# shg8/3DGS.cpp

Hardware: AMD Instinct MI355X
Metric: frames/sec at 1920×1080, 1M Gaussians (higher is better)
Workload: dtype f32

## Files before the change

### 3dgs.cpp_amd/binding.py

```python
import ctypes as C
import os

import numpy as np

_HERE = os.path.dirname(os.path.abspath(__file__))
LIB_PATH = os.environ.get("GS3D_HIP_LIB", os.path.join(_HERE, "libgs3d_hip.so"))

UNIFORMS_DT = np.dtype([("camera_position", "<f4", 4), ("proj_mat", "<f4", 16), ("view_mat", "<f4", 16),
                        ("width", "<u4"), ("height", "<u4"), ("tan_fovx", "<f4"), ("tan_fovy", "<f4")])
CAMERA_DT = np.dtype([("position", "<f4", 3), ("rotation", "<f4", 4), ("fov", "<f4"),
                      ("near_plane", "<f4"), ("far_plane", "<f4")])
VERTEX_FLOATS = 60
RECORD_FLOATS = 62
BLOB_PLANES = 59


KERNEL_SOURCES = ("gs_device.h", "gs_bin.h", "gs_scene.hip", "gs_preprocess.hip", "gs_radix.hip", "gs_bin_l1.hip", "gs_bin_l2.hip",
                  "gs_blend.hip", "gs_kernels.h")


def library_source_hash():
    import hashlib
    import re
    h = hashlib.sha256()
# ... 7 lines not shown
            text = re.sub(r"#[^\n]*", " ", text)
        h.update(name.encode() + b"\0" + " ".join(text.split()).encode())
    return h.hexdigest()


STAGES = dict(tiles=(0, np.uint32), depth=(1, np.float32), radius=(2, np.float32), aabb=(3, np.uint16),
              conic_opacity=(4, np.float32), uv_rg=(5, np.float32), b=(6, np.float32),
              depth_order=(7, np.uint32), alpha_cut=(8, np.float32), sorted_tile=(11, np.uint32), sorted_gid=(12, np.uint32),
              ranges=(13, np.uint32), lists_raw=(14, np.uint32), ranges_raw=(15, np.uint32))

SYMBOLS = ["gs_last_error", "gs_device_count", "gs_read_ply", "gs_activate_records", "gs_scene_load_ply", "gs_scene_from_records",
           "gs_scene_from_vertices", "gs_scene_from_device_blob", "gs_scene_blob_floats", "gs_scene_blob",
           "gs_scene_num_vertices", "gs_scene_quantize_sh", "gs_scene_sh_bits", "gs_scene_download_vertex_range",
           "gs_scene_download_vertices", "gs_scene_download_cov3d",
           "gs_scene_destroy", "gs_renderer_create", "gs_renderer_destroy", "gs_camera_uniforms",
           "gs_render", "gs_render_host", "gs_synchronize", "gs_set_timing", "gs_set_frames_in_flight", "gs_set_sort_path", "gs_set_exp_mode", "gs_set_graph_mode", "gs_set_blend_lockstep", "gs_get_blend_lockstep", "gs_set_blend_contraction", "gs_set_antialiased", "gs_get_antialiased", "gs_get_timing_totals",
           "gs_get_frame_intervals", "gs_get_stats", "gs_poll_stats", "gs_debug_download", "gs_debug_expf_scan", "gs_debug_alpha_cut_scan", "gs_renderer_stream",
           "gs_dist_unique_id", "gs_dist_create", "gs_dist_rank", "gs_dist_world", "gs_dist_pose_count",
           "gs_dist_broadcast_scene", "gs_dist_broadcast_scene_ex", "gs_dist_verify", "gs_dist_destroy"]


class FrameStats(C.Structure):
    _fields_ = [("num_gaussians", C.c_uint64), ("num_visible", C.c_uint64), ("num_instances", C.c_uint64),
                ("instance_capacity", C.c_uint64), ("ms_preprocess", C.c_float), ("ms_prefix_sum", C.c_float),
                ("ms_preprocess_sort", C.c_float), ("ms_sort", C.c_float), ("ms_tile_boundary", C.c_float),
                ("ms_render", C.c_float), ("ms_total", C.c_float), ("retries", C.c_uint32),
                ("num_bin_entries", C.c_uint32), ("max_bin_entries", C.c_uint32), ("sort_path", C.c_uint32),
                ("bin_tiles", C.c_uint32), ("sort_level", C.c_uint32), ("blend_redo", C.c_uint32), ("blend_resolved", C.c_uint32), ("pad_", C.c_uint32)]

    def as_dict(self):
        return {k: getattr(self, k) for k, _ in self._fields_}
# ... 27 lines not shown
    if _LIB is None:
        if not os.path.exists(LIB_PATH):
            raise GsError(-3, f"{LIB_PATH} is missing: run __graft_entry__.build() (hipcc, gfx950)")
        L = C.CDLL(LIB_PATH)
        L.gs_last_error.restype = C.c_char_p
        L.gs_scene_num_vertices.restype = C.c_uint64
        L.gs_scene_num_vertices.argtypes = [C.c_void_p]
        L.gs_scene_blob_floats.restype = C.c_uint64
        L.gs_scene_blob_floats.argtypes = [C.c_uint64]
        L.gs_renderer_stream.restype = C.c_void_p
        L.gs_renderer_stream.argtypes = [C.c_void_p]
        L.gs_scene_destroy.argtypes = [C.c_void_p]
        L.gs_renderer_destroy.argtypes = [C.c_void_p]
        L.gs_scene_destroy.restype = None
        L.gs_renderer_destroy.restype = None
        _LIB = L
    return _LIB


def _check(rc):
    if rc != 0:
        raise GsError(rc, lib().gs_last_error().decode(errors="replace"))


def _p(a):
    if not isinstance(a, np.ndarray) or not a.flags["C_CONTIGUOUS"]:
        raise TypeError("_p() takes a C-contiguous numpy array that the caller keeps alive for the duration of the call")
    return C.c_void_p(a.ctypes.data)


# ... 137 lines not shown

    def set_exp_mode(self, mode):
        _check(lib().gs_set_exp_mode(self._h, C.c_int(int(mode))))

    def set_blend_contraction(self, enabled):
        _check(lib().gs_set_blend_contraction(self._h, C.c_int(int(bool(enabled)))))

    def set_antialiased(self, enabled):
        _check(lib().gs_set_antialiased(self._h, C.c_int(int(bool(enabled)))))

    @property
    def antialiased(self):
        rc = lib().gs_get_antialiased(self._h)
        _check(min(rc, 0))
        return bool(rc)

    def set_fast_blend(self, fast):
        self.set_exp_mode(0 if fast else 2)
        self.set_blend_contraction(bool(fast))

    def set_graph_mode(self, enabled):
        _check(lib().gs_set_graph_mode(self._h, C.c_int(int(bool(enabled)))))

    def set_blend_lockstep(self, mode):
        _check(lib().gs_set_blend_lockstep(self._h, C.c_int(int(mode))))

    def blend_lockstep(self):
        settled = C.c_int(0)
        now = lib().gs_get_blend_lockstep(self._h, C.byref(settled))
        if now < 0:
# ... 105 lines not shown
```

### 3dgs.cpp_amd/csrc/gs_blend.hip

```cpp
#include "gs_device.h"

namespace gs {

#ifndef GS_BLEND_ASM_ACCUMULATE
#define GS_BLEND_ASM_ACCUMULATE 1
#endif
#ifndef GS_BLEND_ASM_LOOP
#define GS_BLEND_ASM_LOOP 1
#endif
#ifndef GS_BLEND_SALU_DIET
#define GS_BLEND_SALU_DIET 2
#endif


__device__ __forceinline__ float min_q_rect(float c00, float c01, float c11, float u, float v, float xa,
                                            float xb, float ya, float yb) {
    const float dx_lo = u - xb, dx_hi = u - xa, dy_lo = v - yb, dy_hi = v - ya;
    const bool in_x = !(dx_lo > 0.0f) && !(dx_hi < 0.0f), in_y = !(dy_lo > 0.0f) && !(dy_hi < 0.0f);
    const float h00 = 0.5f * c00, h11 = 0.5f * c11;
    const float r11 = -c01 * __builtin_amdgcn_rcpf(c11), r00 = -c01 * __builtin_amdgcn_rcpf(c00);
    const float a = dx_lo > 0.0f ? dx_lo : dx_hi;
    const float t = fminf(fmaxf(r11 * a, dy_lo), dy_hi);
    const float qv = __builtin_fmaf(t, __builtin_fmaf(h11, t, c01 * a), h00 * a * a);
    const float b = dy_lo > 0.0f ? dy_lo : dy_hi;
// ... 518 lines not shown
                if (alive == 0) bm = 0;
#endif
            }
        }
        }
        if (alive == 0) break;
        if (GUARD) {
            S += __builtin_fmaf(T_cs * 1.00001f, __builtin_amdgcn_rcpf(T), -1.0f);
            T_cs = T;
        }
    }
    STAT_ADD(7, (unsigned long long)__popcll(alive) * (range.y - range.x));
    return !abandon;
}

template <int EXP, bool CONTRACT, bool GUARD>
__global__ __launch_bounds__(BLOCK) __attribute__((amdgpu_waves_per_eu(8, 8))) void k_blend(const uint2* __restrict__ ranges,
                                                 const uint32_t* __restrict__ sorted_gid,
                                                 const uint32_t* __restrict__ tile_order,
                                                 const AttrRecord* __restrict__ rec,
                                                 uint32_t width, uint32_t height, uint32_t tiles_x,
                                                 float4* __restrict__ rgba, uchar4* __restrict__ bgra,
                                                 Counters* __restrict__ counters, Counters* host_counters,
                                                 const FrameParams* __restrict__ fp, uint32_t* __restrict__ vis_count, uint32_t lockstep,
                                                 uint64_t* __restrict__ stamps) {
    frame_stamp(stamps, ST_BLEND);
#if defined(GS_BLEND_STATS) || defined(GS_BLEND_CLOCK)
    const long long stat_c0 = clock64();
    const unsigned long long stat_w0 = wall_clock64();
#endif
    static_assert(!GUARD || (EXP != 2 && !CONTRACT), "the guard belongs to a fast exp on the uncontracted arithmetic");
    if (fp) {
        rgba = reinterpret_cast<float4*>(fp->rgba);
        bgra = reinterpret_cast<uchar4*>(fp->bgra);
        host_counters = fp->host_counters;
    }
    __shared__ float4 s_rec[4][3][WAVE];
    __shared__ uint2 s_exptab[(EXP == 2 || GUARD) ? 4 : 1][32];
    __shared__ uint32_t s_klist[GUARD ? 4 : 1][GUARD ? kGuardList : 1];

    const int tid = threadIdx.x, lane = tid & (WAVE - 1), w = tid / WAVE;
    if (EXP == 2) {
        if (lane < 32) {
            const uint64_t v = kExpfTab[lane];
            s_exptab[w][lane] = make_uint2((uint32_t)v, (uint32_t)(v >> 32));
        }
        __builtin_amdgcn_wave_barrier();
    }
    if (host_counters && blockIdx.x == 0 && tid == 0) *host_counters = *counters;
    if (vis_count && blockIdx.x == 0 && (uint32_t)tid < kVisRegions) {
// ... 39 lines not shown
        if ((threadIdx.x & (WAVE - 1)) == 0 && slot < kClockSlots)
            g_blend_clock[slot] = make_uint2((uint32_t)(clock64() - stat_c0), (uint32_t)(wall_clock64() - stat_w0));
    }
#endif
    if (inside) {
        const size_t p = (size_t)py * width + px;
        if (rgba) rgba[p] = make_float4(c0, c1, c2, 1.0f);
        if (bgra) {
            const float r = fminf(fmaxf(c0, 0.0f), 1.0f), g = fminf(fmaxf(c1, 0.0f), 1.0f),
                        b = fminf(fmaxf(c2, 0.0f), 1.0f);
            bgra[p] = make_uchar4((unsigned char)(int)__builtin_rintf(b * 255.0f),
                                  (unsigned char)(int)__builtin_rintf(g * 255.0f),
                                  (unsigned char)(int)__builtin_rintf(r * 255.0f), 255);
        }
    }
}

template <int EXP, bool CONTRACT, bool GUARD>
static void launch_blend_as(const uint32_t* ranges, const uint32_t* sorted_gid, const uint32_t* tile_order, const AttrView& av,
                            uint32_t width, uint32_t height, uint32_t tx, uint32_t ty, float* rgba, uint8_t* bgra,
                            Counters* counters, Counters* host_counters, const FrameParams* fp, bool lockstep, uint64_t* stamps, hipStream_t s) {
    hipLaunchKernelGGL((k_blend<EXP, CONTRACT, GUARD>), dim3(tx * ty), dim3(BLOCK), 0, s, reinterpret_cast<const uint2*>(ranges),
                       sorted_gid, tile_order, av.rec, width, height, tx, reinterpret_cast<float4*>(rgba),
                       reinterpret_cast<uchar4*>(bgra), counters, host_counters, fp, av.vis_count, lockstep ? 1u : 0u, stamps);
}

__global__ __launch_bounds__(WAVE) void k_frame_end(uint64_t* __restrict__ stamps, uint64_t* host_stamps, const FrameParams* __restrict__ fp) {
    if (fp) host_stamps = fp->host_stamps;
    const uint64_t now = wall_clock64();
    const int t = threadIdx.x;
    if (t < ST_COUNT) {
        const uint64_t v = t == ST_END ? now : stamps[t];
        if (t == ST_END) stamps[t] = now;
        if (host_stamps) host_stamps[t] = v;
    }
}
void launch_frame_end(uint64_t* stamps, uint64_t* host_stamps, const FrameParams* fp, hipStream_t s) {
    if (!stamps) return;
    hipLaunchKernelGGL(k_frame_end, dim3(1), dim3(WAVE), 0, s, stamps, host_stamps, fp);
}

void launch_blend(const uint32_t* ranges, const uint32_t* sorted_gid, const uint32_t* tile_order, const AttrView& av,
                  uint32_t width,
                  uint32_t height, float* rgba, uint8_t* bgra, Counters* counters,
                  Counters* host_counters, int exp_mode, bool contract, const FrameParams* fp, bool lockstep, uint64_t* stamps, hipStream_t s) {
    if (width == 0 || height == 0) return;
    const uint32_t tx = (width + kTile - 1) / kTile, ty = (height + kTile - 1) / kTile;
    if (exp_mode == 3 && !contract)
        return launch_blend_as<1, false, true>(ranges, sorted_gid, tile_order, av, width, height, tx, ty, rgba, bgra, counters,
                                               host_counters, fp, lockstep, stamps, s);
    if (exp_mode == 3) exp_mode = 1;
#define GS_BLEND_CASE(E, C)                                                                                              \
    if (exp_mode == E && contract == C)                                                                                  \
        return launch_blend_as<E, C, false>(ranges, sorted_gid, tile_order, av, width, height, tx, ty, rgba, bgra,       \
                                            counters, host_counters, fp, lockstep, stamps, s)
    GS_BLEND_CASE(0, true);
    GS_BLEND_CASE(0, false);
    GS_BLEND_CASE(1, true);
    GS_BLEND_CASE(1, false);
    GS_BLEND_CASE(2, true);
    GS_BLEND_CASE(2, false);
#undef GS_BLEND_CASE
}


__global__ __launch_bounds__(BLOCK) void k_expf_scan(uint32_t first_bits, uint64_t count, unsigned long long* __restrict__ block_sums,
                                                     unsigned long long* __restrict__ guard_max ) {
    const uint64_t base = (uint64_t)blockIdx.x << 20;
    unsigned long long sum = 0;
    double worst = 0.0, worst_near = 0.0;
// ... 76 lines not shown
```

### 3dgs.cpp_amd/csrc/gs_kernels.h

```cpp
#pragma once
#include <hip/hip_runtime.h>
#include <stdint.h>

#include "../../include/gs3d_hip.h"

namespace gs {

constexpr int kTile = 16;
constexpr int kSortTileKeys = 2048;
constexpr int kSortMaxBlocks = 1024;

enum ScenePlane { P_POS = 0, P_SCALE = 3, P_ROT = 6, P_OPACITY = 10, P_SH = 11, P_COUNT = 59 };
constexpr uint64_t blob_stride(uint64_t n) { return (n + 15) & ~uint64_t(15); }
constexpr uint64_t blob_floats(uint64_t n) { return P_SH * blob_stride(n) + 48 * n; }

struct SceneView {
    const float* blob;
    const float* cov3d;
    uint32_t n;
    uint32_t stride;
    const uint16_t* sh16;
    const float* acut;
    const uint32_t* perm;
};
// ... 16 lines not shown
    uint32_t vis_region_slots;
};
constexpr uint32_t kVisRegions = 256, kVisCounterStride = 32;
uint32_t vis_region_slots(uint32_t n);

struct Counters {
    uint32_t visible;
    uint32_t instances;
    uint32_t overflow;
    uint32_t bin_entries;
    uint32_t max_bin;
    uint32_t slabs;
    uint32_t blend_resolved;
    uint32_t blend_redo;
    uint32_t q_head, q_bins_done;
};
enum FrameStamp { ST_PREPROCESS = 0, ST_ORDER = 1, ST_L1_COUNT = 2, ST_L1_SCATTER = 3, ST_L2 = 4, ST_BLEND = 5, ST_END = 6, ST_COUNT = 8 };

struct FrameParams {
    gs_uniforms u;
    float* rgba;
    uint8_t* bgra;
    Counters* host_counters;
    uint64_t* host_stamps;
};

constexpr int kBinSortLevels = 5;
constexpr int kBinSlabLevel = 4;
constexpr uint32_t kBinSortLimit[kBinSortLevels] = {4096, 8192, 12288, 16384, 65535};
constexpr int kBinSortMax = 16384;
constexpr uint32_t kSlabDescBytes = 288, kSlabCapacity = 8192, kSlabWorkGroups = 512, kQueueWorkGroups = 256;

void launch_cov3d(const float* blob, float* cov3d, uint32_t n, uint32_t stride, hipStream_t s);
void launch_alpha_cut(const float* blob, float* cut, uint32_t n, uint32_t stride, uint32_t* beyond_unit, hipStream_t s);
void launch_permute_blob(const float* src, const uint32_t* perm, float* dst, uint32_t n, uint32_t stride, hipStream_t s);
void launch_blob_checksum(const float* blob, uint64_t floats, uint64_t* out, hipStream_t s);
void launch_sh_to_half(const float* blob, uint16_t* sh16, uint32_t n, uint32_t stride, hipStream_t s);
void launch_preprocess(const SceneView& sv, const gs_uniforms& u, const AttrView& av, Counters* counters,
                       const FrameParams* fp, uint64_t* stamps, bool antialiased, hipStream_t s);
// ... 50 lines not shown
void bin_debug_occupancy();
hipError_t bin_prepare_device();
void launch_bin_level1_count(const BinLaunch& b, hipStream_t s);
void launch_bin_level1_scatter(const BinLaunch& b, bool any_order, hipStream_t s);
void launch_bin_level2(const BinLaunch& b, int level, hipStream_t s);

void launch_blend(const uint32_t* ranges, const uint32_t* sorted_gid, const uint32_t* tile_order, const AttrView& av,
                  uint32_t width,
                  uint32_t height, float* rgba, uint8_t* bgra, Counters* counters,
                  Counters* host_counters ,
                  int exp_mode ,
                  bool contract ,
                  const FrameParams* fp,
                  bool lockstep ,
                  uint64_t* stamps ,
                  hipStream_t s);

}
```

### 3dgs.cpp_amd/csrc/gs_preprocess.hip

```cpp
#include "gs_device.h"

namespace gs {

#ifndef GS_PRE_AA_BISECT
#define GS_PRE_AA_BISECT 0
#endif

#ifndef GS_PRE_SH_LDS
#define GS_PRE_SH_LDS 1
#endif

constexpr float SH_C0 = 0.28209479177387814f;
constexpr float SH_C1 = 0.4886025119029199f;

__device__ __forceinline__ float ndc2pix(float v, int S) { return ((v + 1.0f) * (float)S - 1.0f) * 0.5f; }

struct PreUniforms {
    gs_uniforms u;
    Counters* counters;
    const FrameParams* fp;
    uint64_t* stamps;
};

constexpr int kPrePlane = 68, kPreStage = 3 * kPrePlane + 16;
// ... 324 lines not shown
    __shared__ float4 s_stage[BLOCK / WAVE][kPreWaveLds];
    const gs_uniforms& u = pu.fp ? pu.fp->u : pu.u;
    const uint32_t i = blockIdx.x * BLOCK + threadIdx.x;
    frame_stamp(pu.stamps, ST_PREPROCESS);
    if (i == 0 && pu.counters) {
        pu.counters->visible = 0;
        pu.counters->instances = 0;
        pu.counters->overflow = 0;
        pu.counters->bin_entries = 0;
        pu.counters->max_bin = 0;
        pu.counters->slabs = 0;
        pu.counters->blend_resolved = 0;
        pu.counters->blend_redo = 0;
        pu.counters->q_head = 0;
        pu.counters->q_bins_done = 0;
    }
    preprocess_one<AA>(sv, u, av, i, i < sv.n, s_stage[threadIdx.x / WAVE]);
}

void launch_preprocess(const SceneView& sv, const gs_uniforms& u, const AttrView& av, Counters* counters,
                       const FrameParams* fp, uint64_t* stamps, bool antialiased, hipStream_t s) {
    if (sv.n == 0) return;
    PreUniforms pu;
    pu.u = u;
    pu.counters = counters;
    pu.fp = fp;
    pu.stamps = stamps;
    if (antialiased)
        hipLaunchKernelGGL(k_preprocess<true>, dim3((sv.n + BLOCK - 1) / BLOCK), dim3(BLOCK), 0, s, sv, pu, av);
    else
// ... 4 lines not shown
```

### 3dgs.cpp_amd/csrc/gs_renderer.cpp

```cpp
#include <algorithm>
#include <chrono>
#include <cstdio>
#include <cstdlib>
#include <cstring>
#include <limits>
#include <memory>
#include <string>
#include <vector>

#include "gs_blend_tuner.h"
#include "gs_internal.h"

using namespace gs_host;

#ifndef GS_L1_DENSE
#define GS_L1_DENSE 1
#endif
struct FrameBuffers {
    hipStream_t stream = nullptr;
    hipStream_t blend_stream = nullptr;
    hipEvent_t prep_done = nullptr, blend_done = nullptr;
    bool blend_recorded = false;
    DevBuf<uint32_t> tiles;
    DevBuf<float> depth;
    DevBuf<ushort4> aabb;
    DevBuf<gs::AttrRecord> rec;
    DevBuf<uint4> vis;
    DevBuf<uint32_t> vis_count;
    bool planes_stale = false;
    uint32_t vis_region_slots = 0;
    DevBuf<uint32_t> dkeys[2], dvals[2];
    DevBuf<uint32_t> block_hist, digit_total;
    DevBuf<uint32_t> l1_hist, bin_count;
    DevBuf<uint32_t> cand;
    DevBuf<uint32_t> sorted;
// ... 14 lines not shown
                   capacity == o.capacity && cand_capacity == o.cand_capacity && tile_order == o.tile_order && ranges == o.ranges && sh16 == o.sh16;
        }
    } graph_keys[2];
    void drop_graph(int which) {
        if (graph_execs[which]) (void)hipGraphExecDestroy(graph_execs[which]);
        graph_execs[which] = nullptr;
        graph_keys[which] = GraphKey{};
    }
    void drop_graph() {
        drop_graph(0);
        drop_graph(1);
    }
    size_t n = 0;
    bool ready = false;

    void init(size_t n_, uint32_t capacity, uint32_t cand_capacity, const std::vector<uint32_t>& mask_prep, const std::vector<uint32_t>& mask_blend, bool dense_lists) {
        n = n_;
        if (!mask_prep.empty() && !mask_blend.empty()) {
            HIP_CHECK(hipExtStreamCreateWithCUMask(&stream, static_cast<uint32_t>(mask_prep.size()), mask_prep.data()));
            HIP_CHECK(hipExtStreamCreateWithCUMask(&blend_stream, static_cast<uint32_t>(mask_blend.size()), mask_blend.data()));
            HIP_CHECK(hipEventCreateWithFlags(&prep_done, hipEventDisableTiming));
            HIP_CHECK(hipEventCreateWithFlags(&blend_done, hipEventDisableTiming));
        } else {
            HIP_CHECK(hipStreamCreateWithFlags(&stream, hipStreamNonBlocking));
        }
        tiles.alloc(n);
        depth.alloc(n);
        aabb.alloc(n);
        rec.alloc(n);
        vis_region_slots = gs::vis_region_slots(static_cast<uint32_t>(n));
        if (dense_lists) ensure_dense_lists();
        l1_hist.alloc(1025 * static_cast<size_t>(gs::bin_level1_columns(static_cast<uint32_t>(n))));
        bin_count.alloc(2048);
        counters.alloc(1);
        stamps.alloc(gs::ST_COUNT);
        HIP_CHECK(hipMemset(stamps.p, 0, gs::ST_COUNT * sizeof(uint64_t)));
        params.alloc(1);
        set_capacity(capacity);
        set_cand_capacity(cand_capacity);
        ready = true;
// ... 15 lines not shown
    }
    void set_capacity(uint32_t cap) {
        drop_graph();
        sorted.alloc(static_cast<size_t>(cap) + 4);
    }
    void set_cand_capacity(uint32_t ccap) {
        drop_graph();
        cand.alloc(3 * static_cast<size_t>(ccap));
        HIP_CHECK(hipMemset(cand.p, 0, 3 * static_cast<size_t>(ccap) * sizeof(uint32_t)));
    }
    void sync() const {
        HIP_CHECK(hipStreamSynchronize(stream));
        if (blend_stream) HIP_CHECK(hipStreamSynchronize(blend_stream));
    }
    ~FrameBuffers() {
        drop_graph();
        if (stream) (void)hipStreamDestroy(stream);
        if (blend_stream) (void)hipStreamDestroy(blend_stream);
        if (prep_done) (void)hipEventDestroy(prep_done);
        if (blend_done) (void)hipEventDestroy(blend_done);
    }
};

struct FrameSlot {
    gs_uniforms u{};
    float* rgba = nullptr;
    uint8_t* bgra = nullptr;
    hipEvent_t done = nullptr;
    gs::Counters* h_counters = nullptr;
    uint64_t* h_stamps = nullptr;
    gs::FrameParams* h_params = nullptr;
    bool timed = false;
    int level = 0;
    int bin_shift = 3;
    bool lockstep = false;
    uint32_t tune_round = 0;
    int tune_shape = 0;
};

struct gs_renderer {
    static constexpr int kMaxInFlight = 8;
    static constexpr int kSlots = 2 * kMaxInFlight;

    gs_scene* scene = nullptr;
    bool timing = true;
// ... 12 lines not shown

    gs_frame_stats last{};

    int sort_mode = 0;
    int level = 0;
    uint32_t frames_since_fallback = 0;
    uint32_t slab_hold = 32, slab_clean_frames = 0;
    static constexpr int kGlobalLevel = gs::kBinSortLevels;
    static uint32_t level_limit(int lv) { return gs::kBinSortLimit[lv]; }
    int frame_level() const { return sort_mode == 1 ? kGlobalLevel : level; }
    bool graph_mode = false;
    int exp_mode = 3;
    int blend_exp_mode() const { return exp_mode == 3 && !contract && !scene->unit_opacity ? 2 : exp_mode; }
    bool contract = false;
    bool antialiased = false;
    BlendTunerBank tuners;
    int min_bin_shift = 3;
    uint64_t dense_min = 4u << 20;
    bool debug_levels = std::getenv("GS_DEBUG_LEVELS") != nullptr;
    bool level2_queue = !(std::getenv("GS_L2_QUEUE") && std::atoi(std::getenv("GS_L2_QUEUE")) == 0);
    double stall_ms = std::getenv("GS_DEBUG_STALLS") ? std::atof(std::getenv("GS_DEBUG_STALLS")) : 0.0;
    static constexpr int kLaps = 10;
    std::chrono::steady_clock::time_point laps[kLaps];
    void lap(int k) {
        if (stall_ms > 0.0) laps[k] = std::chrono::steady_clock::now();
    }
    void report_stall() {
        if (stall_ms <= 0.0) return;
        auto ms = [&](int a, int b) { return std::chrono::duration<double, std::milli>(laps[b] - laps[a]).count(); };
        if (ms(0, 9) < stall_ms) return;
// ... 7 lines not shown
    uint32_t retries = 0;
    uint32_t redo_chain = 0;
    double total_ms[7] = {0, 0, 0, 0, 0, 0, 0};
    uint64_t total_frames = 0;
    uint64_t lifetime_frames = 0;
    static constexpr size_t kIntervalRing = 8192;
    std::vector<float> intervals;
    bool prev_retired = false;
    uint64_t latest_done = 0;

    uint32_t* sorted_gid = nullptr;
    uint32_t* depth_order = nullptr;
    uint64_t num_tiles = 0;

    ~gs_renderer() {
        for (auto& sl : slots) {
            if (sl.done) (void)hipEventDestroy(sl.done);
            if (sl.h_counters) (void)hipHostFree(sl.h_counters);
            if (sl.h_stamps) (void)hipHostFree(sl.h_stamps);
            if (sl.h_params) (void)hipHostFree(sl.h_params);
        }
    }

    void set_capacity(uint32_t cap) {
        capacity = cap;
        for (auto& fb : sets)
            if (fb.ready) fb.set_capacity(cap);
    }
    void set_cand_capacity(uint32_t ccap) {
        cand_capacity = ccap;
// ... 14 lines not shown
            HIP_CHECK(hipEventCreateWithFlags(&sl.done, hipEventDisableTiming));
            HIP_CHECK(hipHostMalloc(reinterpret_cast<void**>(&sl.h_stamps), gs::ST_COUNT * sizeof(uint64_t), hipHostMallocDefault));
            std::memset(sl.h_stamps, 0, gs::ST_COUNT * sizeof(uint64_t));
            HIP_CHECK(hipHostMalloc(reinterpret_cast<void**>(&sl.h_counters), sizeof(gs::Counters), hipHostMallocDefault));
            *sl.h_counters = gs::Counters{};
            HIP_CHECK(hipHostMalloc(reinterpret_cast<void**>(&sl.h_params), sizeof(gs::FrameParams), hipHostMallocDefault));
        }
        uint64_t want = std::max<uint64_t>(1u << 20, 8 * static_cast<uint64_t>(scene->n));
        if (const char* e = std::getenv("GS_INITIAL_CAPACITY")) want = std::max<uint64_t>(256, std::strtoull(e, nullptr, 10));
        capacity = static_cast<uint32_t>(std::min<uint64_t>(want, kMaxInstances));
        uint64_t want_cand = std::max<uint64_t>(1u << 18, 2 * static_cast<uint64_t>(scene->n));
        if (const char* e = std::getenv("GS_INITIAL_CAND_CAPACITY")) want_cand = std::max<uint64_t>(256, std::strtoull(e, nullptr, 10));
        else if (std::getenv("GS_INITIAL_CAPACITY")) want_cand = std::min<uint64_t>(want_cand, want);
        cand_capacity = static_cast<uint32_t>(std::min<uint64_t>(want_cand, capacity));
        parse_cu_masks();
        sets[0].init(scene->n, capacity, cand_capacity, mask_prep, mask_blend, scene->n >= dense_min);
    }

    std::vector<uint32_t> mask_prep, mask_blend;
    static std::vector<uint32_t> parse_mask(const char* hex) {
        std::vector<uint32_t> words;
        if (!hex) return words;
        std::string h(hex);
        while (h.size() % 8) h.insert(h.begin(), '0');
        for (size_t i = h.size(); i >= 8; i -= 8) words.push_back(static_cast<uint32_t>(std::stoul(h.substr(i - 8, 8), nullptr, 16)));
        return words;
    }
    void parse_cu_masks() {
        mask_prep = parse_mask(std::getenv("GS_CU_MASK_PREP"));
        mask_blend = parse_mask(std::getenv("GS_CU_MASK_BLEND"));
    }

    void set_num_sets(int k) {
        for (int i = 0; i < k; ++i)
            if (!sets[i].ready) sets[i].init(scene->n, capacity, cand_capacity, mask_prep, mask_blend, scene->n >= dense_min);
        num_sets = k;
    }

    DevBuf<uint32_t> tile_order;
    uint32_t order_tx = 0, order_ty = 0;
    void ensure_tile_order(uint32_t tx, uint32_t ty) {
        if (tx == order_tx && ty == order_ty && tile_order.p) return;
        drain();
        constexpr uint32_t B = 4;
        const uint64_t nt = static_cast<uint64_t>(tx) * ty;
        std::vector<std::vector<uint32_t>> per_xcd(8);
        const uint32_t nbx = (tx + B - 1) / B, nby = (ty + B - 1) / B;
        for (uint32_t by = 0; by < nby; ++by)
            for (uint32_t bx = 0; bx < nbx; ++bx) {
                auto& list = per_xcd[(bx + 3 * by) % 8];
// ... 75 lines not shown
        const bool bin_local = lv < kGlobalLevel;
        num_tiles = nt;
        ensure_tile_order(tx, ty);
        lap(2);

        gs::SceneView sv{scene->render_blob(), scene->cov3d.p, n, static_cast<uint32_t>(gs::blob_stride(n)),
                          scene->sh_half ? scene->sh16.p : nullptr, scene->acut.p, scene->perm.p};
        gs::Counters* cnt = fb.counters.p;
        const bool l1_any_order = bin_local && geo.bin_shift <= 3;
        const bool dense_list = GS_L1_DENSE && l1_any_order && n != 0 && n >= dense_min && fb.vis.p && u.width != 0 && u.height != 0;
        gs::AttrView av{fb.tiles.p, fb.depth.p, fb.aabb.p, fb.rec.p, dense_list ? fb.vis.p : nullptr, dense_list ? fb.vis_count.p : nullptr,
                        fb.vis_region_slots};
        fb.planes_stale = dense_list;

        const bool fused_counters = n != 0 && u.width != 0 && u.height != 0;
        if (!fused_counters) {
            HIP_CHECK(hipMemsetAsync(cnt, 0, sizeof(gs::Counters), stream));
            HIP_CHECK(hipMemsetAsync(fb.ranges.p, 0, 2 * nt * sizeof(uint32_t), stream));
        }
        if (fb.blend_stream && fb.blend_recorded) HIP_CHECK(hipStreamWaitEvent(stream, fb.blend_done, 0));
        uint64_t* const stamps = fb.stamps.p;
        auto passes = [&](const gs::FrameParams* fp, hipStream_t bstream) {
            gs::launch_preprocess(sv, u, av, cnt, fp, stamps, antialiased, stream);
            lap(3);
            if (!bin_local && n != 0) {
                const int blocks = std::max(1, std::min<int>(gs::kSortMaxBlocks, (n + gs::kSortTileKeys - 1) / gs::kSortTileKeys));
                const uint32_t* kin = reinterpret_cast<const uint32_t*>(fb.depth.p);
                const uint32_t* vin = nullptr;
                for (int pass = 0; pass < 4; ++pass) {
                    gs::RadixPass p{};
                    const int dst = pass & 1;
                    p.keys_in = kin;
                    p.vals_in = vin;
                    p.keys_out = fb.dkeys[dst].p;
                    p.vals_out = fb.dvals[dst].p;
                    p.n_in = &cnt->visible;
// ... 45 lines not shown
                b.bins_y = geo.bins_y;
                b.bin_shift = geo.bin_shift;
                b.grid_shift = geo.grid_shift;
                b.stamps = stamps;
                gs::launch_bin_level1_count(b, stream);
                gs::launch_bin_level1_scatter(b, l1_any_order, stream);
                lap(5);
                gs::launch_bin_level2(b, lv, stream);
            }
            lap(6);
            if (bstream != stream) {
                HIP_CHECK(hipEventRecord(fb.prep_done, stream));
                HIP_CHECK(hipStreamWaitEvent(bstream, fb.prep_done, 0));
            }
            gs::launch_blend(fb.ranges.p, fb.sorted.p, tile_order.p, av, u.width, u.height, d_rgba, d_bgra, cnt,
                             fused_counters ? sl.h_counters : nullptr, blend_exp_mode(), contract, fp, lockstep, stamps, bstream);
            gs::launch_frame_end(stamps, sl.h_stamps, fp, bstream);
            lap(7);
        };
        depth_order = bin_local ? nullptr : fb.dvals[1].p;
        sorted_gid = fb.sorted.p;
        hipStream_t bstream = fb.blend_stream ? fb.blend_stream : stream;
        const bool replay = graph_mode && fused_counters && !fb.blend_stream;
        if (replay) {
            *sl.h_params = gs::FrameParams{u, d_rgba, d_bgra, sl.h_counters, sl.h_stamps};
            HIP_CHECK(hipMemcpyAsync(fb.params.p, sl.h_params, sizeof(gs::FrameParams), hipMemcpyHostToDevice, stream));
            FrameBuffers::GraphKey key;
            key.level = lv;
            key.bin_shift = geo.bin_shift;
            key.hw_exp = blend_exp_mode();
            key.contract = contract ? 1 : 0;
            key.antialiased = antialiased;
            key.width = u.width;
            key.height = u.height;
            key.capacity = capacity;
            key.cand_capacity = cand_capacity;
            key.tile_order = tile_order.p;
            key.ranges = fb.ranges.p;
            key.sh16 = sv.sh16;
            key.lockstep = lockstep;
// ... 153 lines not shown
        st.num_gaussians = scene->n;
        st.num_visible = sl.h_counters->visible;
        st.num_instances = sl.h_counters->instances;
        st.num_bin_entries = sl.h_counters->bin_entries;
        st.max_bin_entries = sl.h_counters->max_bin;
        st.sort_path = sl.level < kGlobalLevel ? 2u : 1u;
        st.sort_level = static_cast<uint32_t>(sl.level);
        st.bin_tiles = 1u << sl.bin_shift;
        st.instance_capacity = capacity;
        const uint64_t* const ts = sl.h_stamps;
        auto span = [&](int a, int b) {
            const int64_t d = static_cast<int64_t>(ts[b] - ts[a]);
            return d > 0 ? static_cast<float>(static_cast<double>(d) * tick_ms) : 0.0f;
        };
        if (sl.timed) st.ms_total = span(gs::ST_PREPROCESS, gs::ST_END);
        if (sl.timed && timing) {
            const bool global = sl.level >= kGlobalLevel;
            st.ms_preprocess = span(gs::ST_PREPROCESS, global ? gs::ST_ORDER : gs::ST_L1_COUNT);
            st.ms_prefix_sum = span(gs::ST_L1_COUNT, gs::ST_L1_SCATTER);
            st.ms_preprocess_sort = span(gs::ST_L1_SCATTER, gs::ST_L2);
            st.ms_sort = (global ? span(gs::ST_ORDER, gs::ST_L1_COUNT) : 0.0f) + span(gs::ST_L2, gs::ST_BLEND);
            st.ms_tile_boundary = 0.0f;
            st.ms_render = span(gs::ST_BLEND, gs::ST_END);
        }
        st.retries = retries;
        last = st;
        have_frame = true;
        const float v[7] = {st.ms_preprocess, st.ms_prefix_sum, st.ms_preprocess_sort, st.ms_sort,
                            st.ms_tile_boundary, st.ms_render, st.ms_total};
        for (int k = 0; k < 7; ++k) total_ms[k] += v[k];
// ... 41 lines not shown
        if (const char* e = std::getenv("GS_ANTIALIASED")) r->antialiased = std::atoi(e) != 0;
        if (const char* e = std::getenv("GS_BIN_SHIFT")) r->min_bin_shift = std::min(5, std::max(2, std::atoi(e)));
        if (const char* e = std::getenv("GS_SORT_PATH")) {
            const int mode = std::atoi(e);
            if (mode < 0 || mode > 2) throw Error(GS_ERR_INVALID, "GS_SORT_PATH must be 0 (auto), 1 (global) or 2 (bin-local)");
            r->sort_mode = mode;
        }
        *out = r.release();
    });
}

void gs_renderer_destroy(gs_renderer* r) {
    if (r)
        for (auto& fb : r->sets)
            if (fb.ready) {
                (void)hipStreamSynchronize(fb.stream);
                if (fb.blend_stream) (void)hipStreamSynchronize(fb.blend_stream);
            }
    delete r;
}

int gs_render(gs_renderer* r, const gs_uniforms* u, float* d_rgba, uint8_t* d_bgra) {
    return guarded([&] {
        if (!r || !u) throw Error(GS_ERR_INVALID, "null argument");
        if (u->width == 0 || u->height == 0) throw Error(GS_ERR_INVALID, "empty framebuffer");
        r->lap(0);
        r->make_room();
        r->lap(1);
        if (r->stall_ms > 0.0)
            for (int k = 2; k < gs_renderer::kLaps; ++k) r->laps[k] = r->laps[1];
        r->enqueue(*u, d_rgba, d_bgra);
// ... 148 lines not shown
int gs_set_antialiased(gs_renderer* r, int enabled) {
    return guarded([&] {
        if (!r) throw Error(GS_ERR_INVALID, "renderer is null");
        r->drain();
        r->antialiased = enabled != 0;
    });
}

int gs_get_antialiased(gs_renderer* r) {
    int on = 0;
    const int rc = guarded([&] {
        if (!r) throw Error(GS_ERR_INVALID, "renderer is null");
        on = r->antialiased ? 1 : 0;
    });
    return rc != 0 ? rc : on;
}

int gs_set_blend_lockstep(gs_renderer* r, int mode) {
    return guarded([&] {
        if (!r) throw Error(GS_ERR_INVALID, "null argument");
        if (mode < -1 || mode > 1) throw Error(GS_ERR_INVALID, "blend lockstep: -1 automatic, 0 off, 1 on");
        r->drain();
        r->tuners.pin(mode);
    });
}

int gs_get_blend_lockstep(gs_renderer* r, int* settled) {
    int now = 0;
    const int rc = guarded([&] {
        if (!r) throw Error(GS_ERR_INVALID, "null argument");
// ... 87 lines not shown
                    uint64_t pos = 0;
                    for (uint64_t t = 0; t < nt; ++t)
                        for (uint64_t i = rg[2 * t]; i < rg[2 * t + 1] && pos < d; ++i)
                            out[pos++] = stage == GS_STAGE_SORTED_GID ? lists[i] : static_cast<uint32_t>(t);
                    return;
                }
            case GS_STAGE_LISTS_RAW: src = r->sorted_gid; size = d * 4; break;
            case GS_STAGE_RANGES_RAW: src = r->last_set->ranges.p; size = r->num_tiles * 8; break;
            default: throw Error(GS_ERR_INVALID, "unknown stage");
        }
        if (bytes < size) throw Error(GS_ERR_INVALID, "destination too small for stage buffer");
        if (size) HIP_CHECK(hipMemcpy(dst, src, size, hipMemcpyDeviceToHost));
    });
}

void* gs_renderer_stream(gs_renderer* r) { return r ? r->sets[0].stream : nullptr; }

}
```

### include/gs3d_hip.h

```cpp
#ifndef GS3D_HIP_H
#define GS3D_HIP_H

#include <stdint.h>

#ifdef __cplusplus
extern "C" {
#endif

typedef struct gs_scene gs_scene;
typedef struct gs_renderer gs_renderer;

enum gs_status {
    GS_OK = 0,
    GS_ERR_INVALID = -1,
    GS_ERR_IO = -2,
    GS_ERR_DEVICE = -3,
    GS_ERR_NOMEM = -4,
    GS_ERR_OVERFLOW = -5
};

typedef struct {
    float position[3];
    float rotation[4];
    float fov;
// ... 82 lines not shown

int gs_camera_uniforms(const gs_camera* cam, uint32_t width, uint32_t height, gs_uniforms* out);

int gs_render(gs_renderer* r, const gs_uniforms* u, float* d_rgba, uint8_t* d_bgra);

int gs_render_host(gs_renderer* r, const gs_uniforms* u, float* h_rgba, uint8_t* h_bgra);

int gs_synchronize(gs_renderer* r);
int gs_set_timing(gs_renderer* r, int enabled);
int gs_set_frames_in_flight(gs_renderer* r, int frames);
int gs_set_sort_path(gs_renderer* r, int mode);
int gs_set_exp_mode(gs_renderer* r, int mode);
int gs_set_blend_contraction(gs_renderer* r, int enabled);
int gs_set_antialiased(gs_renderer* r, int enabled);
int gs_get_antialiased(gs_renderer* r);
int gs_set_graph_mode(gs_renderer* r, int enabled);
int gs_set_blend_lockstep(gs_renderer* r, int mode);
int gs_get_blend_lockstep(gs_renderer* r, int* settled);
int gs_get_timing_totals(gs_renderer* r, gs_frame_stats* sum, uint64_t* frames, int reset);
int gs_get_frame_intervals(gs_renderer* r, float* out_ms, uint64_t capacity, uint64_t* n_out, int reset);
int gs_get_stats(gs_renderer* r, gs_frame_stats* out);
int gs_poll_stats(gs_renderer* r, gs_frame_stats* out, uint64_t* frames_retired);
int gs_debug_download(gs_renderer* r, int stage, void* dst, uint64_t bytes);
int gs_debug_expf_scan(int device, uint32_t first_bits, uint64_t count, uint64_t* block_sums, uint64_t blocks_capacity, double* guard);
int gs_debug_alpha_cut_scan(int device, uint32_t first_bits, uint64_t count, uint64_t* mismatches, uint32_t* first_mismatch);
void* gs_renderer_stream(gs_renderer* r);

#define GS_DIST_ID_BYTES 128
typedef struct gs_dist gs_dist;
int gs_dist_unique_id(uint8_t id[GS_DIST_ID_BYTES]);
// ... 24 lines not shown
```

Measured before the change: 4670.

## Fuse frame-end stamp into blend kernel tail and add stream-priority modes

The separate k_frame_end launch after blending is removed by default. The last blend workgroup to exit, detected with a per-block LDS counter plus a global exit counter, now copies the timestamps to the host-mapped buffer and writes a frame tag. This saves one kernel launch and its inter-kernel gap each frame. The tail reads its arguments straight from the kernarg segment at a fixed offset, which is fragile, and every block now pays an extra atomic. The change also adds optional high/low-priority stream modes, off by default, that let preprocessing of the next frame overlap blending.

```diff
diff --git a/3dgs.cpp_amd/binding.py b/3dgs.cpp_amd/binding.py
--- a/3dgs.cpp_amd/binding.py
+++ b/3dgs.cpp_amd/binding.py
@@ -45,7 +45,7 @@
            "gs_scene_num_vertices", "gs_scene_quantize_sh", "gs_scene_sh_bits", "gs_scene_download_vertex_range",
            "gs_scene_download_vertices", "gs_scene_download_cov3d",
            "gs_scene_destroy", "gs_renderer_create", "gs_renderer_destroy", "gs_camera_uniforms",
-           "gs_render", "gs_render_host", "gs_synchronize", "gs_set_timing", "gs_set_frames_in_flight", "gs_set_sort_path", "gs_set_exp_mode", "gs_set_graph_mode", "gs_set_blend_lockstep", "gs_get_blend_lockstep", "gs_set_blend_contraction", "gs_set_antialiased", "gs_get_antialiased", "gs_get_timing_totals",
+           "gs_render", "gs_render_host", "gs_synchronize", "gs_set_timing", "gs_set_frames_in_flight", "gs_set_sort_path", "gs_set_exp_mode", "gs_set_graph_mode", "gs_set_blend_lockstep", "gs_get_blend_lockstep", "gs_set_blend_contraction", "gs_set_antialiased", "gs_get_antialiased", "gs_set_stream_priorities", "gs_get_stream_priorities", "gs_debug_frame_end_checks", "gs_get_timing_totals",
            "gs_get_frame_intervals", "gs_get_stats", "gs_poll_stats", "gs_debug_download", "gs_debug_expf_scan", "gs_debug_alpha_cut_scan", "gs_renderer_stream",
            "gs_dist_unique_id", "gs_dist_create", "gs_dist_rank", "gs_dist_world", "gs_dist_pose_count",
            "gs_dist_broadcast_scene", "gs_dist_broadcast_scene_ex", "gs_dist_verify", "gs_dist_destroy"]
@@ -103,6 +103,7 @@
         L.gs_renderer_destroy.argtypes = [C.c_void_p]
         L.gs_scene_destroy.restype = None
         L.gs_renderer_destroy.restype = None
+        L.gs_set_stream_priorities.argtypes = [C.c_void_p, C.c_int]
         _LIB = L
     return _LIB
 
@@ -270,6 +271,20 @@
         rc = lib().gs_get_antialiased(self._h)
         _check(min(rc, 0))
         return bool(rc)
+
+    def set_stream_priorities(self, mode):
+        _check(lib().gs_set_stream_priorities(self._h, C.c_int(int(mode))))
+
+    @property
+    def stream_priorities(self):
+        rc = lib().gs_get_stream_priorities(self._h)
+        _check(min(rc, 0))
+        return int(rc)
+
+    def frame_end_checks(self):
+        out = np.zeros(3, np.uint64)
+        _check(lib().gs_debug_frame_end_checks(self._h, _p(out)))
+        return int(out[0]), int(out[1]), int(out[2])
 
     def set_fast_blend(self, fast):
         self.set_exp_mode(0 if fast else 2)
diff --git a/3dgs.cpp_amd/csrc/gs_blend.hip b/3dgs.cpp_amd/csrc/gs_blend.hip
--- a/3dgs.cpp_amd/csrc/gs_blend.hip
+++ b/3dgs.cpp_amd/csrc/gs_blend.hip
@@ -556,8 +556,31 @@
     return !abandon;
 }
 
+struct BlendEnd {
+    uint64_t* stamps;
+    uint64_t* host_stamps;
+    uint64_t frame_tag;
+    Counters* counters;
+    const FrameParams* fp;
+    uint32_t workgroups;
+};
+struct BlendArgLayout {
+    const void *ranges, *sorted_gid, *tile_order, *rec;
+    uint32_t width, height, tiles_x;
+    void *rgba, *bgra, *counters, *host_counters;
+    const void* fp;
+    void* vis_count;
+    uint32_t lockstep;
+    BlendEnd end;
+};
+constexpr uint32_t kBlendEndOffset = 104;
+static_assert(offsetof(BlendArgLayout, end) == kBlendEndOffset, "k_blend's tail reads its arguments at this offset");
+
+#ifndef GS_BLEND_WAVES
+#define GS_BLEND_WAVES 8
+#endif
 template <int EXP, bool CONTRACT, bool GUARD>
-__global__ __launch_bounds__(BLOCK) __attribute__((amdgpu_waves_per_eu(8, 8))) void k_blend(const uint2* __restrict__ ranges,
+__global__ __launch_bounds__(BLOCK) __attribute__((amdgpu_waves_per_eu(GS_BLEND_WAVES, GS_BLEND_WAVES))) void k_blend(const uint2* __restrict__ ranges,
                                                  const uint32_t* __restrict__ sorted_gid,
                                                  const uint32_t* __restrict__ tile_order,
                                                  const AttrRecord* __restrict__ rec,
@@ -565,8 +588,8 @@
                                                  float4* __restrict__ rgba, uchar4* __restrict__ bgra,
                                                  Counters* __restrict__ counters, Counters* host_counters,
                                                  const FrameParams* __restrict__ fp, uint32_t* __restrict__ vis_count, uint32_t lockstep,
-                                                 uint64_t* __restrict__ stamps) {
-    frame_stamp(stamps, ST_BLEND);
+                                                 const BlendEnd end) {
+    if (end.stamps && blockIdx.x == 0 && threadIdx.x == 0) __hip_atomic_store(&end.stamps[ST_BLEND], wall_clock64(), __ATOMIC_RELAXED, __HIP_MEMORY_SCOPE_AGENT);
 #if defined(GS_BLEND_STATS) || defined(GS_BLEND_CLOCK)
     const long long stat_c0 = clock64();
     const unsigned long long stat_w0 = wall_clock64();
@@ -576,6 +599,13 @@
         rgba = reinterpret_cast<float4*>(fp->rgba);
         bgra = reinterpret_cast<uchar4*>(fp->bgra);
         host_counters = fp->host_counters;
+    }
+    if (end.stamps && blockIdx.x == 0 && threadIdx.x == 0)
+        __hip_atomic_store(&end.stamps[ST_TAG], fp ? fp->frame_tag : end.frame_tag, __ATOMIC_RELAXED, __HIP_MEMORY_SCOPE_AGENT);
+    __shared__ uint32_t s_waves_out;
+    if (end.host_stamps) {
+        if (threadIdx.x == 0) s_waves_out = 0;
+        __syncthreads();
     }
     __shared__ float4 s_rec[4][3][WAVE];
     __shared__ uint2 s_exptab[(EXP == 2 || GUARD) ? 4 : 1][32];
@@ -645,15 +675,44 @@
                                   (unsigned char)(int)__builtin_rintf(r * 255.0f), 255);
         }
     }
+    const BlendEnd* e;
+    {
+        const uint8_t __attribute__((address_space(4)))* ka = (const uint8_t __attribute__((address_space(4)))*)__builtin_amdgcn_kernarg_segment_ptr();
+        asm volatile("" : "+s"(ka));
+        e = (const BlendEnd*)(const uint8_t*)(ka + kBlendEndOffset);
+    }
+    if (e->host_stamps) {
+        __builtin_amdgcn_fence(__ATOMIC_RELEASE, "workgroup");
+        uint32_t last = 0;
+        if (lane == 0) last = atomicAdd(&s_waves_out, 1u) == BLOCK / WAVE - 1 ? 1u : 0u;
+        if (__builtin_amdgcn_readfirstlane(last)) {
+            Counters* const cnt = e->counters;
+            uint32_t done = 0;
+            if (lane == 0) done = atomicAdd(&cnt->blend_exited, 1u);
+            if ((uint32_t)__builtin_amdgcn_readfirstlane(done) == e->workgroups - 1) {
+                uint64_t* const st = e->stamps;
+                uint64_t* const host = e->fp ? e->fp->host_stamps : e->host_stamps;
+                const uint64_t now = wall_clock64();
+                if (lane < ST_COUNT) {
+                    const uint64_t v = lane == ST_END ? now : __hip_atomic_load(&st[lane], __ATOMIC_RELAXED, __HIP_MEMORY_SCOPE_AGENT);
+                    if (lane == ST_END) st[ST_END] = now;
+                    host[lane] = v;
+                }
+                if (lane == 0) cnt->blend_exited = 0;
+            }
+        }
+    }
 }
 
 template <int EXP, bool CONTRACT, bool GUARD>
 static void launch_blend_as(const uint32_t* ranges, const uint32_t* sorted_gid, const uint32_t* tile_order, const AttrView& av,
                             uint32_t width, uint32_t height, uint32_t tx, uint32_t ty, float* rgba, uint8_t* bgra,
-                            Counters* counters, Counters* host_counters, const FrameParams* fp, bool lockstep, uint64_t* stamps, hipStream_t s) {
+                            Counters* counters, Counters* host_counters, const FrameParams* fp, bool lockstep, uint64_t* stamps,
+                            uint64_t* host_stamps, uint64_t frame_tag, hipStream_t s) {
     hipLaunchKernelGGL((k_blend<EXP, CONTRACT, GUARD>), dim3(tx * ty), dim3(BLOCK), 0, s, reinterpret_cast<const uint2*>(ranges),
                        sorted_gid, tile_order, av.rec, width, height, tx, reinterpret_cast<float4*>(rgba),
-                       reinterpret_cast<uchar4*>(bgra), counters, host_counters, fp, av.vis_count, lockstep ? 1u : 0u, stamps);
+                       reinterpret_cast<uchar4*>(bgra), counters, host_counters, fp, av.vis_count, lockstep ? 1u : 0u,
+                       BlendEnd{stamps, stamps ? host_stamps : nullptr, frame_tag, counters, fp, tx * ty});
 }
 
 __global__ __launch_bounds__(WAVE) void k_frame_end(uint64_t* __restrict__ stamps, uint64_t* host_stamps, const FrameParams* __restrict__ fp) {
@@ -674,17 +733,18 @@
 void launch_blend(const uint32_t* ranges, const uint32_t* sorted_gid, const uint32_t* tile_order, const AttrView& av,
                   uint32_t width,
                   uint32_t height, float* rgba, uint8_t* bgra, Counters* counters,
-                  Counters* host_counters, int exp_mode, bool contract, const FrameParams* fp, bool lockstep, uint64_t* stamps, hipStream_t s) {
+                  Counters* host_counters, int exp_mode, bool contract, const FrameParams* fp, bool lockstep, uint64_t* stamps,
+                  uint64_t* host_stamps, uint64_t frame_tag, hipStream_t s) {
     if (width == 0 || height == 0) return;
     const uint32_t tx = (width + kTile - 1) / kTile, ty = (height + kTile - 1) / kTile;
     if (exp_mode == 3 && !contract)
         return launch_blend_as<1, false, true>(ranges, sorted_gid, tile_order, av, width, height, tx, ty, rgba, bgra, counters,
-                                               host_counters, fp, lockstep, stamps, s);
+                                               host_counters, fp, lockstep, stamps, host_stamps, frame_tag, s);
     if (exp_mode == 3) exp_mode = 1;
 #define GS_BLEND_CASE(E, C)                                                                                              \
     if (exp_mode == E && contract == C)                                                                                  \
         return launch_blend_as<E, C, false>(ranges, sorted_gid, tile_order, av, width, height, tx, ty, rgba, bgra,       \
-                                            counters, host_counters, fp, lockstep, stamps, s)
+                                            counters, host_counters, fp, lockstep, stamps, host_stamps, frame_tag, s)
     GS_BLEND_CASE(0, true);
     GS_BLEND_CASE(0, false);
     GS_BLEND_CASE(1, true);
diff --git a/3dgs.cpp_amd/csrc/gs_kernels.h b/3dgs.cpp_amd/csrc/gs_kernels.h
--- a/3dgs.cpp_amd/csrc/gs_kernels.h
+++ b/3dgs.cpp_amd/csrc/gs_kernels.h
@@ -54,8 +54,9 @@
     uint32_t blend_resolved;
     uint32_t blend_redo;
     uint32_t q_head, q_bins_done;
+    uint32_t blend_exited;
 };
-enum FrameStamp { ST_PREPROCESS = 0, ST_ORDER = 1, ST_L1_COUNT = 2, ST_L1_SCATTER = 3, ST_L2 = 4, ST_BLEND = 5, ST_END = 6, ST_COUNT = 8 };
+enum FrameStamp { ST_PREPROCESS = 0, ST_ORDER = 1, ST_L1_COUNT = 2, ST_L1_SCATTER = 3, ST_L2 = 4, ST_BLEND = 5, ST_END = 6, ST_TAG = 7, ST_COUNT = 8 };
 
 struct FrameParams {
     gs_uniforms u;
@@ -63,6 +64,7 @@
     uint8_t* bgra;
     Counters* host_counters;
     uint64_t* host_stamps;
+    uint64_t frame_tag;
 };
 
 constexpr int kBinSortLevels = 5;
@@ -143,6 +145,8 @@
                   const FrameParams* fp,
                   bool lockstep ,
                   uint64_t* stamps ,
+                  uint64_t* host_stamps ,
+                  uint64_t frame_tag,
                   hipStream_t s);
 
 }
diff --git a/3dgs.cpp_amd/csrc/gs_preprocess.hip b/3dgs.cpp_amd/csrc/gs_preprocess.hip
--- a/3dgs.cpp_amd/csrc/gs_preprocess.hip
+++ b/3dgs.cpp_amd/csrc/gs_preprocess.hip
@@ -362,6 +362,7 @@
         pu.counters->blend_redo = 0;
         pu.counters->q_head = 0;
         pu.counters->q_bins_done = 0;
+        pu.counters->blend_exited = 0;
     }
     preprocess_one<AA>(sv, u, av, i, i < sv.n, s_stage[threadIdx.x / WAVE]);
 }
diff --git a/3dgs.cpp_amd/csrc/gs_renderer.cpp b/3dgs.cpp_amd/csrc/gs_renderer.cpp
--- a/3dgs.cpp_amd/csrc/gs_renderer.cpp
+++ b/3dgs.cpp_amd/csrc/gs_renderer.cpp
@@ -16,9 +16,18 @@
 #ifndef GS_L1_DENSE
 #define GS_L1_DENSE 1
 #endif
+struct StreamPlan {
+    int mode = 0;
+    int high = 0, low = 0;
+    hipStream_t shared_blend = nullptr;
+    std::vector<uint32_t> mask_prep, mask_blend;
+    bool cu_masked() const { return !mask_prep.empty() && !mask_blend.empty(); }
+};
+
 struct FrameBuffers {
     hipStream_t stream = nullptr;
     hipStream_t blend_stream = nullptr;
+    bool owns_blend_stream = false, cu_masked = false;
     hipEvent_t prep_done = nullptr, blend_done = nullptr;
     bool blend_recorded = false;
     DevBuf<uint32_t> tiles;
@@ -63,16 +72,39 @@
     size_t n = 0;
     bool ready = false;
 
-    void init(size_t n_, uint32_t capacity, uint32_t cand_capacity, const std::vector<uint32_t>& mask_prep, const std::vector<uint32_t>& mask_blend, bool dense_lists) {
-        n = n_;
-        if (!mask_prep.empty() && !mask_blend.empty()) {
-            HIP_CHECK(hipExtStreamCreateWithCUMask(&stream, static_cast<uint32_t>(mask_prep.size()), mask_prep.data()));
-            HIP_CHECK(hipExtStreamCreateWithCUMask(&blend_stream, static_cast<uint32_t>(mask_blend.size()), mask_blend.data()));
+    void make_streams(const StreamPlan& plan) {
+        drop_streams();
+        if (plan.cu_masked()) {
+            HIP_CHECK(hipExtStreamCreateWithCUMask(&stream, static_cast<uint32_t>(plan.mask_prep.size()), plan.mask_prep.data()));
+            HIP_CHECK(hipExtStreamCreateWithCUMask(&blend_stream, static_cast<uint32_t>(plan.mask_blend.size()), plan.mask_blend.data()));
+            owns_blend_stream = cu_masked = true;
+        } else if (plan.mode == 0) {
+            HIP_CHECK(hipStreamCreateWithFlags(&stream, hipStreamNonBlocking));
+        } else {
+            HIP_CHECK(hipStreamCreateWithPriority(&stream, hipStreamNonBlocking, plan.high));
+            if (plan.mode == 1) {
+                HIP_CHECK(hipStreamCreateWithPriority(&blend_stream, hipStreamNonBlocking, plan.low));
+                owns_blend_stream = true;
+            } else {
+                blend_stream = plan.shared_blend;
+            }
+        }
+        if (blend_stream && !prep_done) {
             HIP_CHECK(hipEventCreateWithFlags(&prep_done, hipEventDisableTiming));
             HIP_CHECK(hipEventCreateWithFlags(&blend_done, hipEventDisableTiming));
-        } else {
-            HIP_CHECK(hipStreamCreateWithFlags(&stream, hipStreamNonBlocking));
-        }
+        }
+        blend_recorded = false;
+    }
+    void drop_streams() {
+        drop_graph();
+        if (stream) (void)hipStreamDestroy(stream);
+        if (blend_stream && owns_blend_stream) (void)hipStreamDestroy(blend_stream);
+        stream = blend_stream = nullptr;
+        owns_blend_stream = cu_masked = false;
+    }
+    void init(size_t n_, uint32_t capacity, uint32_t cand_capacity, const StreamPlan& plan, bool dense_lists) {
+        n = n_;
+        make_streams(plan);
         tiles.alloc(n);
         depth.alloc(n);
         aabb.alloc(n);
@@ -118,9 +150,7 @@
         if (blend_stream) HIP_CHECK(hipStreamSynchronize(blend_stream));
     }
     ~FrameBuffers() {
-        drop_graph();
-        if (stream) (void)hipStreamDestroy(stream);
-        if (blend_stream) (void)hipStreamDestroy(blend_stream);
+        drop_streams();
         if (prep_done) (void)hipEventDestroy(prep_done);
         if (blend_done) (void)hipEventDestroy(blend_done);
     }
@@ -133,6 +163,7 @@
     hipEvent_t done = nullptr;
     gs::Counters* h_counters = nullptr;
     uint64_t* h_stamps = nullptr;
+    uint64_t tag = 0;
     gs::FrameParams* h_params = nullptr;
     bool timed = false;
     int level = 0;
@@ -175,6 +206,10 @@
     int blend_exp_mode() const { return exp_mode == 3 && !contract && !scene->unit_opacity ? 2 : exp_mode; }
     bool contract = false;
     bool antialiased = false;
+    StreamPlan plan;
+    bool fused_frame_end = !(std::getenv("GS_FRAME_END_KERNEL") && std::atoi(std::getenv("GS_FRAME_END_KERNEL")) != 0);
+    uint64_t end_checked = 0, end_wrong_tag = 0, end_before_blend = 0;
+    uint64_t next_tag = 0;
     BlendTunerBank tuners;
     int min_bin_shift = 3;
     uint64_t dense_min = 4u << 20;
@@ -212,6 +247,8 @@
     uint64_t num_tiles = 0;
 
     ~gs_renderer() {
+        for (auto& fb : sets) fb.drop_streams();
+        if (plan.shared_blend) (void)hipStreamDestroy(plan.shared_blend);
         for (auto& sl : slots) {
             if (sl.done) (void)hipEventDestroy(sl.done);
             if (sl.h_counters) (void)hipHostFree(sl.h_counters);
@@ -256,10 +293,32 @@
         else if (std::getenv("GS_INITIAL_CAPACITY")) want_cand = std::min<uint64_t>(want_cand, want);
         cand_capacity = static_cast<uint32_t>(std::min<uint64_t>(want_cand, capacity));
         parse_cu_masks();
-        sets[0].init(scene->n, capacity, cand_capacity, mask_prep, mask_blend, scene->n >= dense_min);
-    }
-
-    std::vector<uint32_t> mask_prep, mask_blend;
+        HIP_CHECK(hipDeviceGetStreamPriorityRange(&plan.low, &plan.high));
+        if (const char* e = std::getenv("GS_STREAM_PRIORITIES")) {
+            const int mode = std::atoi(e);
+            if (mode < 0 || mode > 2) throw Error(GS_ERR_INVALID, "GS_STREAM_PRIORITIES must be 0 (one stream per set), 1 (per-set blend streams) or 2 (shared blend stream)");
+            plan.mode = mode;
+        }
+        ensure_shared_blend();
+        sets[0].init(scene->n, capacity, cand_capacity, plan, scene->n >= dense_min);
+    }
+    void ensure_shared_blend() {
+        if (plan.mode == 2 && !plan.cu_masked() && !plan.shared_blend)
+            HIP_CHECK(hipStreamCreateWithPriority(&plan.shared_blend, hipStreamNonBlocking, plan.low));
+    }
+    void set_stream_mode(int mode) {
+        for (auto& fb : sets)
+            if (fb.ready) fb.sync();
+        plan.mode = mode;
+        ensure_shared_blend();
+        for (auto& fb : sets)
+            if (fb.ready) fb.make_streams(plan);
+        if (plan.mode != 2 && plan.shared_blend) {
+            (void)hipStreamDestroy(plan.shared_blend);
+            plan.shared_blend = nullptr;
+        }
+    }
+
     static std::vector<uint32_t> parse_mask(const char* hex) {
         std::vector<uint32_t> words;
         if (!hex) return words;
@@ -269,13 +328,13 @@
         return words;
     }
     void parse_cu_masks() {
-        mask_prep = parse_mask(std::getenv("GS_CU_MASK_PREP"));
-        mask_blend = parse_mask(std::getenv("GS_CU_MASK_BLEND"));
+        plan.mask_prep = parse_mask(std::getenv("GS_CU_MASK_PREP"));
+        plan.mask_blend = parse_mask(std::getenv("GS_CU_MASK_BLEND"));
     }
 
     void set_num_sets(int k) {
         for (int i = 0; i < k; ++i)
-            if (!sets[i].ready) sets[i].init(scene->n, capacity, cand_capacity, mask_prep, mask_blend, scene->n >= dense_min);
+            if (!sets[i].ready) sets[i].init(scene->n, capacity, cand_capacity, plan, scene->n >= dense_min);
         num_sets = k;
     }
 
@@ -381,12 +440,13 @@
         fb.planes_stale = dense_list;
 
         const bool fused_counters = n != 0 && u.width != 0 && u.height != 0;
+        if (fb.blend_stream && fb.blend_recorded) HIP_CHECK(hipStreamWaitEvent(stream, fb.blend_done, 0));
         if (!fused_counters) {
             HIP_CHECK(hipMemsetAsync(cnt, 0, sizeof(gs::Counters), stream));
             HIP_CHECK(hipMemsetAsync(fb.ranges.p, 0, 2 * nt * sizeof(uint32_t), stream));
         }
-        if (fb.blend_stream && fb.blend_recorded) HIP_CHECK(hipStreamWaitEvent(stream, fb.blend_done, 0));
         uint64_t* const stamps = fb.stamps.p;
+        sl.tag = ++next_tag;
         auto passes = [&](const gs::FrameParams* fp, hipStream_t bstream) {
             gs::launch_preprocess(sv, u, av, cnt, fp, stamps, antialiased, stream);
             lap(3);
@@ -462,16 +522,17 @@
                 HIP_CHECK(hipStreamWaitEvent(bstream, fb.prep_done, 0));
             }
             gs::launch_blend(fb.ranges.p, fb.sorted.p, tile_order.p, av, u.width, u.height, d_rgba, d_bgra, cnt,
-                             fused_counters ? sl.h_counters : nullptr, blend_exp_mode(), contract, fp, lockstep, stamps, bstream);
-            gs::launch_frame_end(stamps, sl.h_stamps, fp, bstream);
+                             fused_counters ? sl.h_counters : nullptr, blend_exp_mode(), contract, fp, lockstep, stamps,
+                             fused_frame_end ? sl.h_stamps : nullptr, sl.tag, bstream);
+            if (!fused_frame_end) gs::launch_frame_end(stamps, sl.h_stamps, fp, bstream);
             lap(7);
         };
         depth_order = bin_local ? nullptr : fb.dvals[1].p;
         sorted_gid = fb.sorted.p;
-        hipStream_t bstream = fb.blend_stream ? fb.blend_stream : stream;
-        const bool replay = graph_mode && fused_counters && !fb.blend_stream;
+        const bool replay = graph_mode && fused_counters && !fb.cu_masked;
+        hipStream_t bstream = fb.blend_stream && !replay ? fb.blend_stream : stream;
         if (replay) {
-            *sl.h_params = gs::FrameParams{u, d_rgba, d_bgra, sl.h_counters, sl.h_stamps};
+            *sl.h_params = gs::FrameParams{u, d_rgba, d_bgra, sl.h_counters, sl.h_stamps, sl.tag};
             HIP_CHECK(hipMemcpyAsync(fb.params.p, sl.h_params, sizeof(gs::FrameParams), hipMemcpyHostToDevice, stream));
             FrameBuffers::GraphKey key;
             key.level = lv;
@@ -655,6 +716,11 @@
             return d > 0 ? static_cast<float>(static_cast<double>(d) * tick_ms) : 0.0f;
         };
         if (sl.timed) st.ms_total = span(gs::ST_PREPROCESS, gs::ST_END);
+        if (sl.timed) {
+            ++end_checked;
+            if (ts[gs::ST_TAG] != sl.tag) ++end_wrong_tag;
+            if (static_cast<int64_t>(ts[gs::ST_END] - ts[gs::ST_BLEND]) < 0) ++end_before_blend;
+        }
         if (sl.timed && timing) {
             const bool global = sl.level >= kGlobalLevel;
             st.ms_preprocess = span(gs::ST_PREPROCESS, global ? gs::ST_ORDER : gs::ST_L1_COUNT);
@@ -726,7 +792,7 @@
     if (r)
         for (auto& fb : r->sets)
             if (fb.ready) {
-                (void)hipStreamSynchronize(fb.stream);
+                if (fb.stream) (void)hipStreamSynchronize(fb.stream);
                 if (fb.blend_stream) (void)hipStreamSynchronize(fb.blend_stream);
             }
     delete r;
@@ -905,6 +971,36 @@
         on = r->antialiased ? 1 : 0;
     });
     return rc != 0 ? rc : on;
+}
+
+int gs_set_stream_priorities(gs_renderer* r, int mode) {
+    return guarded([&] {
+        if (mode < 0 || mode > 2)
+            throw Error(GS_ERR_INVALID, "stream priorities: 0 (one stream per set), 1 (per-set blend streams) or 2 (shared blend stream)");
+        if (!r) throw Error(GS_ERR_INVALID, "renderer is null");
+        HIP_CHECK(hipSetDevice(r->scene->device));
+        r->drain();
+        if (mode != r->plan.mode) r->set_stream_mode(mode);
+    });
+}
+
+int gs_get_stream_priorities(gs_renderer* r) {
+    int mode = 0;
+    const int rc = guarded([&] {
+        if (!r) throw Error(GS_ERR_INVALID, "renderer is null");
+        mode = r->plan.mode;
+    });
+    return rc != 0 ? rc : mode;
+}
+
+int gs_debug_frame_end_checks(gs_renderer* r, uint64_t* out3) {
+    return guarded([&] {
+        if (!r || !out3) throw Error(GS_ERR_INVALID, "null argument");
+        r->drain();
+        out3[0] = r->end_checked;
+        out3[1] = r->end_wrong_tag;
+        out3[2] = r->end_before_blend;
+    });
 }
 
 int gs_set_blend_lockstep(gs_renderer* r, int mode) {
@@ -1022,6 +1118,10 @@
     });
 }
 
-void* gs_renderer_stream(gs_renderer* r) { return r ? r->sets[0].stream : nullptr; }
-
-}
+void* gs_renderer_stream(gs_renderer* r) {
+    if (!r) return nullptr;
+    const FrameBuffers& fb = r->sets[0];
+    return fb.blend_stream && !(r->graph_mode && !fb.cu_masked) ? fb.blend_stream : fb.stream;
+}
+
+}
diff --git a/include/gs3d_hip.h b/include/gs3d_hip.h
--- a/include/gs3d_hip.h
+++ b/include/gs3d_hip.h
@@ -120,6 +120,9 @@
 int gs_set_blend_contraction(gs_renderer* r, int enabled);
 int gs_set_antialiased(gs_renderer* r, int enabled);
 int gs_get_antialiased(gs_renderer* r);
+int gs_set_stream_priorities(gs_renderer* r, int mode);
+int gs_get_stream_priorities(gs_renderer* r);
+int gs_debug_frame_end_checks(gs_renderer* r, uint64_t* out3);
 int gs_set_graph_mode(gs_renderer* r, int enabled);
 int gs_set_blend_lockstep(gs_renderer* r, int mode);
 int gs_get_blend_lockstep(gs_renderer* r, int* settled);
```

Measured after the change: 4629. No clear change (-0.9%).
